# yjpark1/multiagent_rl

Measured on AMD Instinct MI355X. Metric: env-steps/sec, simple_spread N=6 x B envs, 1/2/4/8 MI355X, higher is better.
Workload: dtype f32

## Files before the change

multiagent_rl_amd/csrc/pw_kernels_spread_quad.hpp:

```cpp
#pragma once

#include "pw_kernels_spread.hpp"

namespace {

__device__ __forceinline__ void quad_pair_of(const int q, int &i, int &j)
{
    i = q < 5 ? 0 : q < 9 ? 1 : q < 12 ? 2 : q < 14 ? 3 : 4;
    j = q - (i == 0 ? 0 : i == 1 ? 5 : i == 2 ? 9 : i == 3 ? 12 : 14) + i + 1;
}

__device__ __forceinline__ void quad_act_fetch(const int32_t *row, const uint32_t lane_off, const uint32_t lds_slot, const uint32_t slot_read)
{
    unsigned keep;
    asm volatile("s_mov_b32 %0, m0\n\ts_mov_b32 m0, %3\n\ts_nop 0\n\tglobal_load_lds_dword %1, %2\n\ts_mov_b32 m0, %0"
                 : "=&s"(keep) : "v"(lane_off), "s"(row), "s"(lds_slot), "v"(slot_read) : "memory");
}

template <bool K1>
__device__ __forceinline__ void quad_pair_force(const float2 qi, const float2 qj, const uint32_t near_lo, const uint32_t near_span,
                                                const float dist_min, const float k, const float cf, float &Fx, float &Fy)
{
    const float dx = qi.x - qj.x, dy = qi.y - qj.y;
    const float d2 = dx * dx + dy * dy;
    const f32x2 a = {cf * dx, cf * dy};
    const bool near = __float_as_uint(d2) - near_lo >= near_span;
    const bool uni = (k >= 9.094947017729282e-13f) & (k <= 1099511627776.0f) & (cf >= 9.5367431640625e-07f) & (cf <= 128.0f);
    const bool c1 = (__float_as_uint(d2) - 0x12800000u) < (0x6C800000u - 0x12800000u);
    const bool c2 = fminf(fabsf(a.x), fabsf(a.y)) >= 8.673617379884035e-19f;
    const bool fast = near & c1 & c2 & uni;
    const bool any_cold = __builtin_amdgcn_ballot_w64(near & !fast) != 0;
    Fx = 0.0f; Fy = 0.0f;
    if (fast) {
        const float dist = sqrt_rn_core(d2);
        const float y0 = __builtin_amdgcn_rcpf(dist);
        __builtin_amdgcn_sched_barrier(0);
        const float yd = __builtin_fmaf(__builtin_fmaf(-dist, y0, 1.0f), y0, y0);
        const f32x2 Q = div_chain2(a, dist, yd);
        const float xarg = K1 ? div_chain1(-(dist - dist_min), k, div_refined_rcp(k))
                              : div_chain(-(dist - dist_min), k, div_refined_rcp(k));
        const float pen = softplus_branchless(xarg) * k;
        const f32x2 F = Q * f32x2{pen, pen};
        Fx = F.x;
        Fy = F.y;
    }
    if (__builtin_expect(any_cold, 0)) {
        if (near & !fast) collision_force_pair<true, K1>(qi.x, qi.y, qj.x, qj.y, dist_min, k, cf, Fx, Fy);
    }
}

#ifndef PW_QUAD_BARRIER
#define PW_QUAD_BARRIER(t) duo_barrier()
#endif
#ifndef PW_QUAD_ACT_AHEAD
#define PW_QUAD_ACT_AHEAD 4
#endif
#ifndef PW_QUAD_PAD_P
#define PW_QUAD_PAD_P()
#endif
#ifndef PW_QUAD_PAD_OB
#define PW_QUAD_PAD_OB()
#endif
constexpr int kQuadActAhead = PW_QUAD_ACT_AHEAD;
constexpr int kQuadN = 6, kQuadL = 6, kQuadEPP = 4, kQuadEPW = 8;
struct SpreadQuadLds { float4 *s_ring; float2 *s_ftab, *s_lmB, *s_utab; float *s_min, *s_rew; int32_t *s_act; uint32_t bytes; };
__host__ __device__ inline SpreadQuadLds spread_quad_lds(unsigned char *raw = nullptr)
{
    LdsCursor c{reinterpret_cast<float *>(raw)}; SpreadQuadLds o;
    o.s_ring = c.take<float4>(4 * kWave);
    o.s_ftab = c.take<float2>(2 * kQuadEPP * kQuadN * kQuadN);
    o.s_min = c.take<float>(kWave); o.s_rew = c.take<float>(kWave);
    o.s_lmB = c.take<float2>(kQuadEPW * kQuadL); o.s_act = c.take<int32_t>(2 * kQuadActAhead * kWave);
    o.s_utab = c.take<float2>(2 * 8);
    o.bytes = 4 * c.at; return o;
}
template <bool UNIT_MASS, bool COLL = false, bool K1 = false>
__global__ void __launch_bounds__(4 * kWave) pw_spread_quad_kernel(const StreamParams A, const int T)
{
    constexpr int N = kQuadN, L = kQuadL, D = 16, P2 = 15, EPP = kQuadEPP, EPW = kQuadEPW;
    extern __shared__ __attribute__((aligned(16))) unsigned char smem_raw[];
    const SpreadQuadLds Y = spread_quad_lds(smem_raw);

    const int wave = __builtin_amdgcn_readfirstlane((((int)threadIdx.x >> 6) + 2 * (((int)blockIdx.x >> 8) & 1)) & 3);
    const int lane = (int)threadIdx.x & 63;
    const int env0 = (int)blockIdx.x * EPW;
    const int envs_here = A.B - env0 < EPW ? A.B - env0 : EPW;
    const size_t BN = (size_t)A.B * N;

    const bool resets = A.auto_reset && A.max_episode_len > 0;
    int offs_all = A.ep_step[env0 + (lane < envs_here ? lane : 0)];
    auto next_reset_step = [&](int t_from) -> int {
        if (!resets) return 0x7fffffff;
        int rem = A.max_episode_len - 1 - (t_from + offs_all);
        rem = rem < 0 ? 0 : rem;
        int m = 0x7fffffff;
        for (int e = 0; e < envs_here; ++e) {
            const int r = __builtin_amdgcn_readlane(rem, e);
            m = r < m ? r : m;
        }
        return t_from + m;
    };
    int t_reset = next_reset_step(0);
    auto reset_step_update = [&](int t) {
        if (t + 1 + offs_all >= A.max_episode_len) offs_all = -(t + 1);
        t_reset = next_reset_step(t + 1);
    };
    int cur = 0;

    if (wave < 2) {
        __builtin_amdgcn_s_setprio(3);
        const int e0 = wave * EPP;
        const int nv = envs_here - e0 < 0 ? 0 : envs_here - e0 < EPP ? envs_here - e0 : EPP;
        if (nv == 0) {
            for (int t = 0; t < T; ++t) PW_QUAD_BARRIER(t);
            return;
        }
        const int la = lane < nv * N ? lane : 0;
        const int e4 = la / N, a = la - e4 * N;
        const int me = (e0 + e4) * N + a;
        const int env = env0 + e0 + e4;
        const uint32_t g = (uint32_t)env * (uint32_t)N + (uint32_t)a;
        const uint64_t env_id = A.env_id_base + (uint64_t)env;
        const int lp = lane < nv * P2 ? lane : 0;
        const int pe = lp / P2, pq = lp - pe * P2;
        int pi, pj;
        quad_pair_of(pq, pi, pj);
        const int ri = (e0 + pe) * N + pi, rj = (e0 + pe) * N + pj;
        float2 *ftab = Y.s_ftab + wave * (EPP * N * N);
        float2 *f_ij = ftab + (pe * N + pi) * N + (pj - 1), *f_ji = ftab + (pe * N + pj) * N + pi;
        const float2 *row = ftab + (e4 * N + a) * N;

        float px = A.pos_x[g], py = A.pos_y[g], vx = A.vel_x[g], vy = A.vel_y[g];
        int ep_off = A.ep_step[env];
        uint32_t ep_count = A.ep_count[env];
        Y.s_ring[me] = make_float4(px, py, vx, vy);
        float2 *utab = Y.s_utab + wave * 8;
        if (lane < 6) {
            const int ai = lane;
            float ux = 0.0f + ((ai == 1 ? 1.0f : 0.0f) - (ai == 2 ? 1.0f : 0.0f));
            float uy = 0.0f + ((ai == 3 ? 1.0f : 0.0f) - (ai == 4 ? 1.0f : 0.0f));
            ux *= A.sens; uy *= A.sens;
            if (A.fscale != 1.0f) { ux = A.fscale * ux; uy = A.fscale * uy; }
            utab[lane] = make_float2(ux + 0.0f, uy + 0.0f);
        }
        wave_lds_sync();
        const float k = A.contact_margin, cf = A.contact_force, dt = A.dt, damp = A.damp, mass = A.mass;
        const uint32_t near_lo = __float_as_uint(A.near_thr2), near_span = 0x7F800000u - near_lo;
        const unsigned char *act_row = reinterpret_cast<const unsigned char *>(A.act);
        const size_t act_stride = BN * sizeof(int32_t);
        const uint32_t act_off = g * (uint32_t)sizeof(int32_t);
        int32_t *act_ring = Y.s_act + wave * (kQuadActAhead * kWave);
        const uint32_t act_lds = __builtin_amdgcn_readfirstlane((uint32_t)reinterpret_cast<uintptr_t>(act_ring));
        auto fetch_act = [&](int t, uint32_t slot_read) {
            quad_act_fetch(reinterpret_cast<const int32_t *>(act_row), act_off, act_lds + (uint32_t)(t & (kQuadActAhead - 1)) * (kWave * 4), slot_read);
            act_row += t + 1 < T ? act_stride : (size_t)0;
        };
        asm volatile("" :: "v"(ep_off), "v"(ep_count), "v"(offs_all), "v"(px), "v"(py), "v"(vx), "v"(vy), "s"(t_reset));
        for (int t0 = 0; t0 < kQuadActAhead; ++t0) fetch_act(t0, 0u);
        float2 qi = *reinterpret_cast<const float2 *>(Y.s_ring + ri);
        float2 qj = *reinterpret_cast<const float2 *>(Y.s_ring + rj);
        PW_STAMP_DECL;
        for (int t = 0; t < T; ++t) {
            PW_STAMP_START;
            asm volatile("s_waitcnt vmcnt(%0)" :: "n"(kQuadActAhead - 1) : "memory");
            PW_STAMP(3);
            const uint32_t ai = (uint32_t)act_ring[(t & (kQuadActAhead - 1)) * kWave + lane];
            fetch_act(t + kQuadActAhead, ai);
            const float2 u0 = utab[ai < 5u ? ai : 5u];
            const bool two_slots = t == t_reset;
            float Fx, Fy;
            quad_pair_force<K1>(qi, qj, near_lo, near_span, A.dist_min, k, cf, Fx, Fy);
            *f_ij = make_float2(Fx, Fy);
            *f_ji = make_float2(-Fx, -Fy);
            PW_STAMP(0);
            float fx = u0.x, fy = u0.y;
            asm volatile("" ::: "memory");
#pragma unroll
            for (int j = 0; j < N - 1; ++j) {
                const float2 F = row[j];
                fx = F.x + fx;
                fy = F.y + fy;
            }
            vx = vx * damp; vy = vy * damp;
            vx = vx + div_mass<UNIT_MASS>(fx, mass) * dt;
            vy = vy + div_mass<UNIT_MASS>(fy, mass) * dt;
            px = px + vx * dt;
            py = py + vy * dt;
            int nxt = (cur + 1) & 3;
            Y.s_ring[nxt * kWave + me] = make_float4(px, py, vx, vy);
            if (__builtin_expect(two_slots, 0)) {
                if (t + 1 + ep_off >= A.max_episode_len) {
                    ep_count += 1;
                    ep_off = -(t + 1);
                    pw_reset_xy(A.seed, env_id, ep_count, (uint32_t)a, -1.0f, 1.0f, &px, &py);
                    vx = 0.f; vy = 0.f;
                }
                reset_step_update(t);
                nxt = (nxt + 1) & 3;
                Y.s_ring[nxt * kWave + me] = make_float4(px, py, vx, vy);
            }
            cur = nxt;
            asm volatile("" ::: "memory");
            qi = *reinterpret_cast<const float2 *>(Y.s_ring + cur * kWave + ri);
            qj = *reinterpret_cast<const float2 *>(Y.s_ring + cur * kWave + rj);
            PW_STAMP(1);
            PW_QUAD_PAD_P();
            PW_QUAD_BARRIER(t);
            PW_STAMP(2);
        }
        act_fetch_drain();
#ifdef PW_STAMPS
        if (blockIdx.x == 0 && wave == 0 && lane == 0)
            for (int i_ = 0; i_ < 4; ++i_) g_pw_stamps[i_] = st_acc[i_];
#endif
        A.pos_x[g] = px; A.pos_y[g] = py;
        A.vel_x[g] = vx; A.vel_y[g] = vy;
        A.ep_step[env] = T + ep_off;
        A.ep_count[env] = ep_count;
        return;
    }

    int e_local = lane / N;
    int a = lane - e_local * N;
    if (e_local >= envs_here) { e_local = 0; a = 0; }
    const int env = env0 + e_local;
    const int base = e_local * N, me = base + a;
    const uint32_t g = (uint32_t)env * (uint32_t)N + (uint32_t)a;
    const uint64_t env_id = A.env_id_base + (uint64_t)env;
    int ep_off = A.ep_step[env];
    uint32_t ep_count = A.ep_count[env];
    float olx = A.lm_x[(size_t)env * L + a], oly = A.lm_y[(size_t)env * L + a];

    if (wave == 2) {
        float own_p = 0.0f;
        int cnt_p = 0;
        uint32_t cmask_p = 0;
        float2 mine, q6[N];
        auto a_reads = [&](const int nxt) __attribute__((always_inline)) {
            const float4 *slot = Y.s_ring + nxt * kWave + base;
            mine = *reinterpret_cast<const float2 *>(slot + a);
#pragma unroll
            for (int j = 0; j < N; ++j) q6[j] = *reinterpret_cast<const float2 *>(slot + j);
        };
        float best, e0;
        int cnt;
        uint32_t cmask;
        auto a_dist = [&]() __attribute__((always_inline)) {
            const float px = mine.x, py = mine.y;
            float e2[N];
            cnt = 0; cmask = 0;
#pragma unroll
            for (int j = 0; j < N; ++j) {
                const float2 q = q6[j];
                const float dx = q.x - px, dy = q.y - py;
                const float d2 = dx * dx + dy * dy;
                cnt += d2 < A.coll_thr2 ? 1 : 0;
                if (COLL) cmask |= d2 < A.coll_thr2 ? 1u << j : 0u;
                const float ex = q.x - olx, ey = q.y - oly;
                e2[j] = ex * ex + ey * ey;
            }
            best = __builtin_fminf(__builtin_fminf(__builtin_fminf(e2[0], e2[1]), __builtin_fminf(e2[2], e2[3])),
                                   __builtin_fminf(e2[4], e2[5]));
            e0 = e2[0];
        };
        auto a_sqrt = [&]() __attribute__((always_inline)) -> float {
            const float b = e0 != e0 ? e0 : best;
            return sqrtf(b);
        };
        auto a_clock = [&](const int t, int nxt) __attribute__((always_inline)) {
            if (__builtin_expect(t == t_reset, 0)) {
                if (t + 1 + ep_off >= A.max_episode_len) {
                    ep_count += 1;
                    ep_off = -(t + 1);
                    pw_reset_xy(A.seed, env_id, ep_count, (uint32_t)(N + a), -1.0f, 1.0f, &olx, &oly);
                }
                reset_step_update(t);
                nxt = (nxt + 1) & 3;
            }
            cur = nxt;
        };
        float sh_own[L], sh_r[N], r;
        auto b_shfl_own = [&]() __attribute__((always_inline)) {
#pragma unroll
            for (int l = 0; l < L; ++l) sh_own[l] = __shfl(own_p, base + l, kWave);
        };
        auto b_reward = [&]() __attribute__((always_inline)) {
            r = 0.0f;
#pragma unroll
            for (int l = 0; l < L; ++l) r -= sh_own[l];
#pragma unroll
            for (int k2 = 0; k2 < N; ++k2) r -= k2 < cnt_p ? 1.0f : 0.0f;
#pragma unroll
            for (int i = 0; i < N; ++i) sh_r[i] = __shfl(r, base + i, kWave);
        };
        float *rew_t = A.rew, *rsh_t = A.rew_shared;
        uint64_t *coll_t = A.coll;
        auto b_store = [&]() __attribute__((always_inline)) {
            float acc = 0.0f;
#pragma unroll
            for (int i = 0; i < N; ++i) acc += sh_r[i];
            nt_store(rew_t + g, r);
            nt_store(rsh_t + env, acc);
            if (COLL) nt_store(coll_t + g, (uint64_t)cmask_p);
            rew_t += BN; rsh_t += A.B;
            if (COLL) coll_t += BN;
        };
        PW_STAMP_DECL;
        {
            PW_STAMP_START;
            PW_QUAD_BARRIER(0);
            PW_STAMP(0);
            const int nxt = (cur + 1) & 3;
            a_reads(nxt);
            a_dist();
            own_p = a_sqrt(); cnt_p = cnt; cmask_p = cmask;
            a_clock(0, nxt);
            PW_STAMP(1);
        }
        for (int t = 1; t < T; ++t) {
            PW_STAMP_START;
            PW_QUAD_BARRIER(t);
            PW_STAMP(0);
            const int nxt = (cur + 1) & 3;
            a_reads(nxt);
            b_shfl_own();
            a_dist();
            b_reward();
            const float own = a_sqrt();
            b_store();
            own_p = own; cnt_p = cnt; cmask_p = cmask;
            a_clock(t, nxt);
            PW_STAMP(1);
        }
        b_shfl_own();
        b_reward();
        b_store();
#ifdef PW_STAMPS
        if (blockIdx.x == 0 && lane == 0)
            for (int i_ = 0; i_ < 2; ++i_) g_pw_stamps[4 + i_] = st_acc[i_];
#endif
        return;
    }

    const int rows_here = envs_here * N;
    const int cgrp = lane & 3;
    const bool col0 = cgrp == 0;
    int row_u[3];
    uint32_t off_u[3];
#pragma unroll
    for (int u = 0; u < 3; ++u) {
        const int r = (lane >> 2) + 16 * u;
        const bool ok = r < rows_here;
        row_u[u] = ok ? r : 0;
        off_u[u] = (uint32_t)(ok ? lane + 64 * u : cgrp) * 16u;
    }
    float4 lm_u[3];
    auto load_landmarks = [&]() {
#pragma unroll
        for (int u = 0; u < 3; ++u)
            lm_u[u] = *reinterpret_cast<const float4 *>(Y.s_lmB + (row_u[u] / N) * L + (cgrp > 0 ? 2 * cgrp - 2 : 0));
    };
    Y.s_lmB[me] = make_float2(olx, oly);
    wave_lds_sync();
    load_landmarks();
    unsigned char *obs_t = reinterpret_cast<unsigned char *>(A.obs + ((size_t)env0 * N) * D);
    uint8_t *done_t = A.done, *term_t = A.terminal;
    const size_t obs_stride = BN * D * sizeof(float);
    const bool has_len = A.max_episode_len > 0;
    int t_term = has_len ? A.max_episode_len - 1 - ep_off : 0x7fffffff;
    PW_STAMP_DECL;
    for (int t = 0; t < T; ++t) {
        PW_STAMP_START;
        nt_store(done_t + g, (uint8_t)0);
        PW_QUAD_BARRIER(t);
        PW_STAMP(0);
        int nxt = (cur + 1) & 3;
        nt_store(term_t + env, (uint8_t)(t >= t_term ? 1 : 0));
        if (t == t_reset) {
            const bool rst = t >= t_term;
            if (rst) {
                if (A.final_obs) {
                    const float4 st = Y.s_ring[nxt * kWave + me];
                    stream_write_obs<L>(A.final_obs + ((size_t)t * BN + g) * D, L, Y.s_lmB + base, st.x, st.y, st.z, st.w);
                }
                ep_count += 1;
                ep_off = -(t + 1);
                t_term = A.max_episode_len - 1 - ep_off;
                pw_reset_xy(A.seed, env_id, ep_count, (uint32_t)(N + a), -1.0f, 1.0f, &olx, &oly);
            }
            reset_step_update(t);
            wave_lds_sync();
            if (rst) Y.s_lmB[me] = make_float2(olx, oly);
            wave_lds_sync();
            load_landmarks();
            nxt = (nxt + 1) & 3;
        }
        cur = nxt;
        const float4 *slot = Y.s_ring + nxt * kWave;
        float4 st[3];
#pragma unroll
        for (int u = 0; u < 3; ++u) st[u] = slot[row_u[u]];
        asm volatile("" :: "v"(st[0].x), "v"(st[0].y), "v"(st[0].z), "v"(st[0].w), "v"(st[1].x), "v"(st[1].y), "v"(st[1].z),
                           "v"(st[1].w), "v"(st[2].x), "v"(st[2].y), "v"(st[2].z), "v"(st[2].w));
#pragma unroll
        for (int u = 0; u < 3; ++u) {
            const float4 d = make_float4(lm_u[u].x - st[u].x, lm_u[u].y - st[u].y, lm_u[u].z - st[u].x, lm_u[u].w - st[u].y);
            const float4 o = make_float4(col0 ? st[u].z : d.x, col0 ? st[u].w : d.y, col0 ? st[u].x : d.z, col0 ? st[u].y : d.w);
            nt_store(reinterpret_cast<float4 *>(obs_t + off_u[u]), o);
        }
        obs_t += obs_stride; done_t += BN; term_t += A.B;
        PW_QUAD_PAD_OB();
        PW_STAMP(1);
    }
#ifdef PW_STAMPS
    if (blockIdx.x == 0 && lane == 0)
        for (int i_ = 0; i_ < 2; ++i_) g_pw_stamps[6 + i_] = st_acc[i_];
#endif
    A.lm_x[(size_t)env * L + a] = olx;
    A.lm_y[(size_t)env * L + a] = oly;
}

}
```

Baseline: 7.816 billion.

## Move quad-kernel barrier into the physics step and ballot collision masks

Physics waves now record pairwise collision bits as a 64-bit ballot into LDS while computing pair forces, so reward waves popcount the mask instead of recomputing six agent distances per step. The per-step barrier is moved from the end of the physics step to just after the force-row reads (MEET=2, with a partial lgkmcnt wait), which changes how physics and reward/obs waves meet. Extra barriers are added before and after the loop to keep the counts matched. The cost is more complex cross-wave synchronisation and parity-indexed mask slots that must line up with reset handling.

```diff
diff --git a/multiagent_rl_amd/csrc/pw_kernels_spread_quad.hpp b/multiagent_rl_amd/csrc/pw_kernels_spread_quad.hpp
--- a/multiagent_rl_amd/csrc/pw_kernels_spread_quad.hpp
+++ b/multiagent_rl_amd/csrc/pw_kernels_spread_quad.hpp
@@ -17,12 +17,17 @@
                  : "=&s"(keep) : "v"(lane_off), "s"(row), "s"(lds_slot), "v"(slot_read) : "memory");
 }
 
-template <bool K1>
+template <bool K1, bool BALLOT>
 __device__ __forceinline__ void quad_pair_force(const float2 qi, const float2 qj, const uint32_t near_lo, const uint32_t near_span,
-                                                const float dist_min, const float k, const float cf, float &Fx, float &Fy)
+                                                const float dist_min, const float k, const float cf, float &Fx, float &Fy,
+                                                const float coll_thr2, uint64_t *coll_slot)
 {
     const float dx = qi.x - qj.x, dy = qi.y - qj.y;
     const float d2 = dx * dx + dy * dy;
+    if constexpr (BALLOT) {
+        *coll_slot = __builtin_amdgcn_ballot_w64(d2 < coll_thr2);
+        asm volatile("" ::: "memory");
+    }
     const f32x2 a = {cf * dx, cf * dy};
     const bool near = __float_as_uint(d2) - near_lo >= near_span;
     const bool uni = (k >= 9.094947017729282e-13f) & (k <= 1099511627776.0f) & (cf >= 9.5367431640625e-07f) & (cf <= 128.0f);
@@ -51,6 +56,15 @@
 
 #ifndef PW_QUAD_BARRIER
 #define PW_QUAD_BARRIER(t) duo_barrier()
+#define PW_QUAD_BARRIER_ROWS(t) asm volatile("s_waitcnt lgkmcnt(5)\n\ts_barrier" ::: "memory")
+#else
+#define PW_QUAD_BARRIER_ROWS(t) PW_QUAD_BARRIER(t)
+#endif
+#ifndef PW_QUAD_MEET
+#define PW_QUAD_MEET 2
+#endif
+#ifndef PW_QUAD_COLL_BALLOT
+#define PW_QUAD_COLL_BALLOT 1
 #endif
 #ifndef PW_QUAD_ACT_AHEAD
 #define PW_QUAD_ACT_AHEAD 4
@@ -61,7 +75,15 @@
 #ifndef PW_QUAD_PAD_OB
 #define PW_QUAD_PAD_OB()
 #endif
+#ifndef PW_QUAD_PAD_OA
+#define PW_QUAD_PAD_OA()
+#endif
 constexpr int kQuadActAhead = PW_QUAD_ACT_AHEAD;
+constexpr int kQuadMeet = PW_QUAD_MEET;
+static_assert(kQuadMeet >= 0 && kQuadMeet <= 2, "PW_QUAD_MEET: 0, 1 or 2");
+#if defined(PW_EXP_BARRIER2) && PW_QUAD_MEET > 0
+#error "PW_EXP_BARRIER2 skips meetings by their index, which the waves number alike only with PW_QUAD_MEET == 0"
+#endif
 constexpr int kQuadN = 6, kQuadL = 6, kQuadEPP = 4, kQuadEPW = 8;
 struct SpreadQuadLds { float4 *s_ring; float2 *s_ftab, *s_lmB, *s_utab; float *s_min, *s_rew; int32_t *s_act; uint32_t bytes; };
 __host__ __device__ inline SpreadQuadLds spread_quad_lds(unsigned char *raw = nullptr)
@@ -80,6 +102,9 @@
     constexpr int N = kQuadN, L = kQuadL, D = 16, P2 = 15, EPP = kQuadEPP, EPW = kQuadEPW;
     extern __shared__ __attribute__((aligned(16))) unsigned char smem_raw[];
     const SpreadQuadLds Y = spread_quad_lds(smem_raw);
+    constexpr int MEET = COLL ? 0 : kQuadMeet;
+    constexpr bool BALLOT = PW_QUAD_COLL_BALLOT && !COLL, MID = MEET > 0, EXTRA = BALLOT || MID;
+    uint64_t *const s_mask = reinterpret_cast<uint64_t *>(Y.s_min);
 
     const int wave = __builtin_amdgcn_readfirstlane((((int)threadIdx.x >> 6) + 2 * (((int)blockIdx.x >> 8) & 1)) & 3);
     const int lane = (int)threadIdx.x & 63;
@@ -113,6 +138,7 @@
         const int nv = envs_here - e0 < 0 ? 0 : envs_here - e0 < EPP ? envs_here - e0 : EPP;
         if (nv == 0) {
             for (int t = 0; t < T; ++t) PW_QUAD_BARRIER(t);
+            if (EXTRA) PW_QUAD_BARRIER(T);
             return;
         }
         const int la = lane < nv * N ? lane : 0;
@@ -159,6 +185,8 @@
         for (int t0 = 0; t0 < kQuadActAhead; ++t0) fetch_act(t0, 0u);
         float2 qi = *reinterpret_cast<const float2 *>(Y.s_ring + ri);
         float2 qj = *reinterpret_cast<const float2 *>(Y.s_ring + rj);
+        uint32_t mask_off = (uint32_t)wave * 8u;
+        auto mask_slot = [&]() { return reinterpret_cast<uint64_t *>(reinterpret_cast<unsigned char *>(s_mask) + mask_off); };
         PW_STAMP_DECL;
         for (int t = 0; t < T; ++t) {
             PW_STAMP_START;
@@ -169,15 +197,24 @@
             const float2 u0 = utab[ai < 5u ? ai : 5u];
             const bool two_slots = t == t_reset;
             float Fx, Fy;
-            quad_pair_force<K1>(qi, qj, near_lo, near_span, A.dist_min, k, cf, Fx, Fy);
+            quad_pair_force<K1, BALLOT>(qi, qj, near_lo, near_span, A.dist_min, k, cf, Fx, Fy, A.coll_thr2, mask_slot());
+            if (BALLOT) {
+                mask_off ^= 16u;
+                asm volatile("" : "+v"(mask_off));
+            }
+            if (MEET == 1) PW_QUAD_BARRIER(t);
             *f_ij = make_float2(Fx, Fy);
             *f_ji = make_float2(-Fx, -Fy);
             PW_STAMP(0);
             float fx = u0.x, fy = u0.y;
             asm volatile("" ::: "memory");
+            float2 Frow[N - 1];
+#pragma unroll
+            for (int j = 0; j < N - 1; ++j) Frow[j] = row[j];
+            if (MEET == 2) PW_QUAD_BARRIER_ROWS(t);
 #pragma unroll
             for (int j = 0; j < N - 1; ++j) {
-                const float2 F = row[j];
+                const float2 F = Frow[j];
                 fx = F.x + fx;
                 fy = F.y + fy;
             }
@@ -205,8 +242,15 @@
             qj = *reinterpret_cast<const float2 *>(Y.s_ring + cur * kWave + rj);
             PW_STAMP(1);
             PW_QUAD_PAD_P();
-            PW_QUAD_BARRIER(t);
+            if (MEET == 0) PW_QUAD_BARRIER(t);
             PW_STAMP(2);
+        }
+        if (EXTRA) {
+            if (BALLOT) {
+                const float dx = qi.x - qj.x, dy = qi.y - qj.y;
+                *mask_slot() = __builtin_amdgcn_ballot_w64(dx * dx + dy * dy < A.coll_thr2);
+            }
+            PW_QUAD_BARRIER(T);
         }
         act_fetch_drain();
 #ifdef PW_STAMPS
@@ -245,9 +289,21 @@
         float best, e0;
         int cnt;
         uint32_t cmask;
-        auto a_dist = [&]() __attribute__((always_inline)) {
+        const int mask_wave = e_local >> 2, mask_shift = (e_local & 3) * P2;
+        uint32_t pairs_of = 0;
+#pragma unroll
+        for (int q = 0; q < P2; ++q) {
+            int i, j;
+            quad_pair_of(q, i, j);
+            pairs_of |= (i == a || j == a) ? 1u << q : 0u;
+        }
+        uint32_t pairs_p = pairs_of;
+        auto mask_count = [&](const int parity, const uint32_t pairs) __attribute__((always_inline)) -> int {
+            const uint64_t m = s_mask[parity * 2 + mask_wave];
+            return __builtin_popcount((uint32_t)(m >> mask_shift) & pairs);
+        };
+        auto a_count6 = [&]() __attribute__((always_inline)) {
             const float px = mine.x, py = mine.y;
-            float e2[N];
             cnt = 0; cmask = 0;
 #pragma unroll
             for (int j = 0; j < N; ++j) {
@@ -256,6 +312,20 @@
                 const float d2 = dx * dx + dy * dy;
                 cnt += d2 < A.coll_thr2 ? 1 : 0;
                 if (COLL) cmask |= d2 < A.coll_thr2 ? 1u << j : 0u;
+            }
+        };
+        auto a_dist = [&]() __attribute__((always_inline)) {
+            float e2[N];
+            if constexpr (BALLOT) {
+                const float dx = mine.x - mine.x, dy = mine.y - mine.y;
+                cnt = dx * dx + dy * dy < A.coll_thr2 ? 1 : 0;
+                cmask = 0;
+            } else {
+                a_count6();
+            }
+#pragma unroll
+            for (int j = 0; j < N; ++j) {
+                const float2 q = q6[j];
                 const float ex = q.x - olx, ey = q.y - oly;
                 e2[j] = ex * ex + ey * ey;
             }
@@ -268,7 +338,12 @@
             return sqrtf(b);
         };
         auto a_clock = [&](const int t, int nxt) __attribute__((always_inline)) {
+            if (BALLOT) pairs_p = pairs_of;
             if (__builtin_expect(t == t_reset, 0)) {
+                if (BALLOT) {
+                    a_count6();
+                    cnt_p = cnt; pairs_p = 0;
+                }
                 if (t + 1 + ep_off >= A.max_episode_len) {
                     ep_count += 1;
                     ep_off = -(t + 1);
@@ -284,12 +359,12 @@
 #pragma unroll
             for (int l = 0; l < L; ++l) sh_own[l] = __shfl(own_p, base + l, kWave);
         };
-        auto b_reward = [&]() __attribute__((always_inline)) {
+        auto b_reward = [&](const int cnt_b) __attribute__((always_inline)) {
             r = 0.0f;
 #pragma unroll
             for (int l = 0; l < L; ++l) r -= sh_own[l];
 #pragma unroll
-            for (int k2 = 0; k2 < N; ++k2) r -= k2 < cnt_p ? 1.0f : 0.0f;
+            for (int k2 = 0; k2 < N; ++k2) r -= k2 < cnt_b ? 1.0f : 0.0f;
 #pragma unroll
             for (int i = 0; i < N; ++i) sh_r[i] = __shfl(r, base + i, kWave);
         };
@@ -306,6 +381,7 @@
             if (COLL) coll_t += BN;
         };
         PW_STAMP_DECL;
+        if (MID) PW_QUAD_BARRIER(0);
         {
             PW_STAMP_START;
             PW_QUAD_BARRIER(0);
@@ -313,6 +389,7 @@
             const int nxt = (cur + 1) & 3;
             a_reads(nxt);
             a_dist();
+            if (BALLOT && MID) cnt += mask_count(1, pairs_of);
             own_p = a_sqrt(); cnt_p = cnt; cmask_p = cmask;
             a_clock(0, nxt);
             PW_STAMP(1);
@@ -323,17 +400,21 @@
             PW_STAMP(0);
             const int nxt = (cur + 1) & 3;
             a_reads(nxt);
+            const int from_mask = BALLOT ? (MID ? mask_count((t + 1) & 1, pairs_of) : mask_count(t & 1, pairs_p)) : 0;
             b_shfl_own();
             a_dist();
-            b_reward();
+            if (BALLOT && MID) cnt += from_mask;
+            b_reward(BALLOT && !MID ? cnt_p + from_mask : cnt_p);
             const float own = a_sqrt();
             b_store();
             own_p = own; cnt_p = cnt; cmask_p = cmask;
             a_clock(t, nxt);
+            PW_QUAD_PAD_OA();
             PW_STAMP(1);
         }
+        if (EXTRA && !MID) PW_QUAD_BARRIER(T);
         b_shfl_own();
-        b_reward();
+        b_reward(BALLOT && !MID ? cnt_p + mask_count(T & 1, pairs_p) : cnt_p);
         b_store();
 #ifdef PW_STAMPS
         if (blockIdx.x == 0 && lane == 0)
@@ -369,6 +450,7 @@
     const bool has_len = A.max_episode_len > 0;
     int t_term = has_len ? A.max_episode_len - 1 - ep_off : 0x7fffffff;
     PW_STAMP_DECL;
+    if (MID) PW_QUAD_BARRIER(0);
     for (int t = 0; t < T; ++t) {
         PW_STAMP_START;
         nt_store(done_t + g, (uint8_t)0);
@@ -412,6 +494,7 @@
         PW_QUAD_PAD_OB();
         PW_STAMP(1);
     }
+    if (EXTRA && !MID) PW_QUAD_BARRIER(T);
 #ifdef PW_STAMPS
     if (blockIdx.x == 0 && lane == 0)
         for (int i_ = 0; i_ < 2; ++i_) g_pw_stamps[6 + i_] = st_acc[i_];
```

Measured after the change: 7.836 billion, median of 6. Within noise of the previous version (+0.3%).
